# LuoweiZhou/VLP

Measured on NVIDIA H100. Metric: image_text_samples_per_sec, higher is better.
Workload: dtype bf16

## Files before the change

vlp_b200/csrc/common.cuh:

```cuda
#pragma once
#include <cuda.h>
#include <cuda_bf16.h>
#include <cuda_runtime.h>
#include <stdint.h>

#include "wgmma.cuh"

namespace vlpk {

__device__ __forceinline__ uint32_t smem_u32(const void* p) {
  return static_cast<uint32_t>(__cvta_generic_to_shared(p));
}

__device__ __forceinline__ uint32_t lane_id() { return threadIdx.x & 31u; }

__device__ __forceinline__ bool elect_one() {
  uint32_t pred = 0;
  asm volatile(
      "{\n\t"
      ".reg .pred P;\n\t"
      "elect.sync _|P, 0xffffffff;\n\t"
      "selp.u32 %0, 1, 0, P;\n\t"
      "}\n"
      : "=r"(pred));
  return pred != 0;
}

__device__ __forceinline__ void mbar_init(uint64_t* bar, uint32_t count) {
  asm volatile("mbarrier.init.shared::cta.b64 [%0], %1;" ::"r"(smem_u32(bar)), "r"(count) : "memory");
}
__device__ __forceinline__ void fence_mbar_init() {
  asm volatile("fence.mbarrier_init.release.cluster;" ::: "memory");
}
__device__ __forceinline__ void fence_proxy_async_smem() {
  asm volatile("fence.proxy.async.shared::cta;" ::: "memory");
}
__device__ __forceinline__ void mbar_arrive_expect_tx(uint64_t* bar, uint32_t bytes) {
  asm volatile("mbarrier.arrive.expect_tx.shared::cta.b64 _, [%0], %1;" ::"r"(smem_u32(bar)), "r"(bytes)
               : "memory");
}
__device__ __forceinline__ void mbar_arrive(uint64_t* bar) {
  asm volatile("mbarrier.arrive.shared::cta.b64 _, [%0];" ::"r"(smem_u32(bar)) : "memory");
}
__device__ __forceinline__ bool mbar_try_wait(uint64_t* bar, uint32_t parity) {
  uint32_t ok;
  asm volatile(
      "{\n\t"
      ".reg .pred P;\n\t"
      "mbarrier.try_wait.parity.shared::cta.b64 P, [%1], %2;\n\t"
      "selp.u32 %0, 1, 0, P;\n\t"
      "}\n"
      : "=r"(ok)
      : "r"(smem_u32(bar)), "r"(parity)
      : "memory");
  return ok != 0;
}
__device__ __forceinline__ void mbar_wait(uint64_t* bar, uint32_t parity) {
  uint32_t spins = 0;
  while (!mbar_try_wait(bar, parity)) {
    if (++spins > (1u << 28)) { __trap(); }
  }
}

__device__ __forceinline__ void pdl_launch_dependents() { asm volatile("griddepcontrol.launch_dependents;" ::: "memory"); }
__device__ __forceinline__ void pdl_wait() { asm volatile("griddepcontrol.wait;" ::: "memory"); }

__device__ __forceinline__ void tma_prefetch_desc(const CUtensorMap* m) {
  asm volatile("prefetch.tensormap [%0];" ::"l"(reinterpret_cast<uint64_t>(m)) : "memory");
}
__device__ __forceinline__ void tma_load_2d(void* dst, const CUtensorMap* m, uint64_t* bar, int c0, int c1) {
  asm volatile(
      "cp.async.bulk.tensor.2d.shared::cluster.global.tile.mbarrier::complete_tx::bytes [%0], [%1, {%3, %4}], [%2];"
      ::"r"(smem_u32(dst)), "l"(reinterpret_cast<uint64_t>(m)), "r"(smem_u32(bar)), "r"(c0), "r"(c1)
      : "memory");
}
__device__ __forceinline__ void tma_load_3d(void* dst, const CUtensorMap* m, uint64_t* bar, int c0, int c1,
                                            int c2) {
  asm volatile(
      "cp.async.bulk.tensor.3d.shared::cluster.global.tile.mbarrier::complete_tx::bytes [%0], [%1, {%3, %4, %5}], "
      "[%2];" ::"r"(smem_u32(dst)),
      "l"(reinterpret_cast<uint64_t>(m)), "r"(smem_u32(bar)), "r"(c0), "r"(c1), "r"(c2)
      : "memory");
}
__device__ __forceinline__ void tma_store_2d(const CUtensorMap* m, const void* src, int c0, int c1) {
  asm volatile("cp.async.bulk.tensor.2d.global.shared::cta.tile.bulk_group [%0, {%2, %3}], [%1];" ::"l"(
                   reinterpret_cast<uint64_t>(m)),
               "r"(smem_u32(src)), "r"(c0), "r"(c1)
               : "memory");
}
__device__ __forceinline__ void tma_store_3d(const CUtensorMap* m, const void* src, int c0, int c1, int c2) {
  asm volatile("cp.async.bulk.tensor.3d.global.shared::cta.tile.bulk_group [%0, {%2, %3, %4}], [%1];" ::"l"(
                   reinterpret_cast<uint64_t>(m)),
               "r"(smem_u32(src)), "r"(c0), "r"(c1), "r"(c2)
               : "memory");
}
__device__ __forceinline__ void tma_reduce_add_2d(const CUtensorMap* m, const void* src, int c0, int c1) {
  asm volatile("cp.reduce.async.bulk.tensor.2d.global.shared::cta.add.tile.bulk_group [%0, {%2, %3}], [%1];" ::"l"(
                   reinterpret_cast<uint64_t>(m)),
               "r"(smem_u32(src)), "r"(c0), "r"(c1)
               : "memory");
}
__device__ __forceinline__ void tma_reduce_add_3d(const CUtensorMap* m, const void* src, int c0, int c1, int c2) {
  asm volatile("cp.reduce.async.bulk.tensor.3d.global.shared::cta.add.tile.bulk_group [%0, {%2, %3, %4}], [%1];" ::"l"(
                   reinterpret_cast<uint64_t>(m)),
               "r"(smem_u32(src)), "r"(c0), "r"(c1), "r"(c2)
               : "memory");
}
__device__ __forceinline__ void tma_store_commit() { asm volatile("cp.async.bulk.commit_group;" ::: "memory"); }
template <int N>
__device__ __forceinline__ void tma_store_wait_read() {
  asm volatile("cp.async.bulk.wait_group.read %0;" ::"n"(N) : "memory");
}
template <int N>
__device__ __forceinline__ void tma_store_wait() {
  asm volatile("cp.async.bulk.wait_group %0;" ::"n"(N) : "memory");
}

__device__ __forceinline__ void wgmma_fence() { asm volatile("wgmma.fence.sync.aligned;" ::: "memory"); }
__device__ __forceinline__ void wgmma_commit() { asm volatile("wgmma.commit_group.sync.aligned;" ::: "memory"); }
template <int N>
__device__ __forceinline__ void wgmma_wait() {
  asm volatile("wgmma.wait_group.sync.aligned %0;" ::"n"(N) : "memory");
}
template <int N>
__device__ __forceinline__ void reg_fence(float (&d)[N]) {
#pragma unroll
  for (int i = 0; i < N; ++i) asm volatile("" : "+f"(d[i])::"memory");
}

__device__ __forceinline__ uint64_t wgmma_desc_sw128(uint32_t saddr, uint32_t lbo_bytes, uint32_t sbo_bytes) {
  uint64_t d = 0;
  d |= static_cast<uint64_t>((saddr & 0x3FFFFu) >> 4);
  d |= static_cast<uint64_t>((lbo_bytes >> 4) & 0x3FFFu) << 16;
  d |= static_cast<uint64_t>((sbo_bytes >> 4) & 0x3FFFu) << 32;
  d |= 1ull << 62;
  return d;
}

__device__ __forceinline__ uint32_t pack_bf16x2(float lo, float hi) {
  __nv_bfloat162 v = __floats2bfloat162_rn(lo, hi);
  return *reinterpret_cast<uint32_t*>(&v);
}
__device__ __forceinline__ float2 unpack_bf16x2(uint32_t u) {
  __nv_bfloat162 v = *reinterpret_cast<__nv_bfloat162*>(&u);
  return __bfloat1622float2(v);
}
__device__ __forceinline__ float bf16_round(float x) { return __bfloat162float(__float2bfloat16_rn(x)); }

__device__ __forceinline__ float fast_ex2(float x) {
  float y;
  asm("ex2.approx.ftz.f32 %0, %1;" : "=f"(y) : "f"(x));
  return y;
}
__device__ __forceinline__ float fast_rcp(float x) {
  float y;
  asm("rcp.approx.ftz.f32 %0, %1;" : "=f"(y) : "f"(x));
  return y;
}

__device__ __forceinline__ void gelu_and_grad(float x, float& g, float& d) {
  const float ax = fabsf(x);
  const float e = fast_ex2(-0.72134752044448170f * x * x);
  const float t = fast_rcp(fmaf(0.3275911f * 0.70710678118654752f, ax, 1.0f));
  float poly = fmaf(1.061405429f, t, -1.453152027f);
  poly = fmaf(poly, t, 1.421413741f);
  poly = fmaf(poly, t, -0.284496736f);
  poly = fmaf(poly, t, 0.254829592f);
  poly *= t;
  const float erf_abs = fmaf(-poly, e, 1.0f);
  const float cdf = 0.5f * (1.0f + copysignf(erf_abs, x));
  g = x * cdf;
  d = fmaf(x * 0.3989422804014327f, e, cdf);
}

struct Philox {
  __device__ __forceinline__ static uint4 gen(uint64_t seed, uint64_t ctr_hi, uint64_t ctr_lo) {
    uint32_t k0 = static_cast<uint32_t>(seed), k1 = static_cast<uint32_t>(seed >> 32);
    uint4 c = make_uint4(static_cast<uint32_t>(ctr_lo), static_cast<uint32_t>(ctr_lo >> 32),
                         static_cast<uint32_t>(ctr_hi), static_cast<uint32_t>(ctr_hi >> 32));
#pragma unroll
    for (int i = 0; i < 10; ++i) {
      const uint32_t hi0 = __umulhi(0xD2511F53u, c.x), lo0 = 0xD2511F53u * c.x;
      const uint32_t hi1 = __umulhi(0xCD9E8D57u, c.z), lo1 = 0xCD9E8D57u * c.z;
      c = make_uint4(hi1 ^ c.y ^ k0, lo1, hi0 ^ c.w ^ k1, lo0);
      k0 += 0x9E3779B9u;
      k1 += 0xBB67AE85u;
    }
    return c;
  }
};
__device__ __forceinline__ uint32_t dropout_keep8(uint64_t seed, uint64_t site, uint64_t idx8, uint32_t thresh16) {
  const uint4 r = Philox::gen(seed, site, idx8);
  uint32_t m = 0;
  m |= ((r.x & 0xFFFFu) >= thresh16) ? 1u : 0u;
  m |= ((r.x >> 16) >= thresh16) ? 2u : 0u;
  m |= ((r.y & 0xFFFFu) >= thresh16) ? 4u : 0u;
  m |= ((r.y >> 16) >= thresh16) ? 8u : 0u;
  m |= ((r.z & 0xFFFFu) >= thresh16) ? 16u : 0u;
  m |= ((r.z >> 16) >= thresh16) ? 32u : 0u;
  m |= ((r.w & 0xFFFFu) >= thresh16) ? 64u : 0u;
  m |= ((r.w >> 16) >= thresh16) ? 128u : 0u;
  return m;
}

struct DropoutCfg {
  float p;
  float scale;
  uint32_t thresh16;
  uint64_t seed;
  uint64_t site;
  const unsigned long long* seed_ptr;
  const unsigned char* bits;
};

__device__ __forceinline__ uint64_t drop_seed(const DropoutCfg& d) {
  return (d.p > 0.f && d.seed_ptr != nullptr) ? d.seed + *d.seed_ptr : d.seed;
}

__host__ inline DropoutCfg make_dropout(float p, uint64_t seed, uint64_t site,
                                        const unsigned long long* seed_ptr = nullptr) {
  DropoutCfg d;
  d.bits = nullptr;
  d.seed_ptr = seed_ptr;
  d.p = p;
  d.scale = p > 0.f ? 1.0f / (1.0f - p) : 1.0f;
  d.thresh16 = static_cast<uint32_t>(p * 65536.0f);
  d.seed = seed;
  d.site = site;
  return d;
}

}
```

vlp_b200/csrc/gemm.cu:

```cuda
#include "gemm.cuh"

#include <cstdlib>

#include "host.cuh"

namespace vlpk {

static constexpr int BM = 128;
static constexpr int BK = 64;
static constexpr int NUM_THREADS = 288;
static constexpr int STG_BYTES = 64 * 128;
static constexpr int SMEM_MAX = 232448;
static constexpr int BN = 128;

struct GemmTmaps {
  CUtensorMap a;
  CUtensorMap b[3];
  CUtensorMap d0;
  CUtensorMap d1;
};

struct GemmArgs {
  int M, N, K;
  int b_seg_rows;
  int splits;
  int split_slices;
  const __nv_bfloat16* bias[3];
  const __nv_bfloat16* aux;
  long long ld_aux;
  float relu_scale;
  DropoutCfg drop;
  float* colsum;
};

template <int STAGES>
struct SmemLayout {
  static constexpr int A_BYTES = BM * BK * 2;
  static constexpr int B_BYTES = BN * BK * 2;
  static constexpr int STAGE_BYTES = A_BYTES + B_BYTES;
  static constexpr int OFF_STG = STAGES * STAGE_BYTES;
  static constexpr int OFF_BAR = OFF_STG + 4 * STG_BYTES;
  static constexpr int NUM_BARS = 2 * STAGES;
  static constexpr int TOTAL = OFF_BAR + NUM_BARS * 8;
  static constexpr int DYN_BYTES = TOTAL + 1024;
  static_assert(DYN_BYTES <= SMEM_MAX, "shared memory budget exceeded");
};

struct StageCount {
  static constexpr int value = (SMEM_MAX - 1024 - 4 * STG_BYTES - 256) / (BM * BK * 2 + BN * BK * 2);
};

__device__ __forceinline__ void wg_bar_sync(int cw) {
  asm volatile("bar.sync %0, 128;" ::"r"(cw + 1) : "memory");
}

template <bool A_MN, bool B_MN, int EPI>
__global__ void __launch_bounds__(NUM_THREADS, 1)
gemm_kernel(const __grid_constant__ GemmTmaps tm, const GemmArgs args) {
  constexpr int STAGES = StageCount::value;
  using L = SmemLayout<STAGES>;
  extern __shared__ uint8_t smem_raw[];
  uint8_t* smem = reinterpret_cast<uint8_t*>((reinterpret_cast<uintptr_t>(smem_raw) + 1023) & ~uintptr_t(1023));

  uint64_t* bars = reinterpret_cast<uint64_t*>(smem + L::OFF_BAR);
  uint64_t* full_bar = bars;
  uint64_t* empty_bar = bars + STAGES;

  pdl_launch_dependents();
  const int wg = threadIdx.x >> 7;
  const int lane = threadIdx.x & 31;

  const int num_m = (args.M + BM - 1) / BM;
  const int num_n = (args.N + BN - 1) / BN;
  const int total_kb = (args.K + BK - 1) / BK;
  const int kb_per = (total_kb + args.splits - 1) / args.splits;
  const int num_work = num_m * num_n * args.splits;

  if (threadIdx.x == 0) {
    tma_prefetch_desc(&tm.a);
    tma_prefetch_desc(&tm.b[0]);
    tma_prefetch_desc(&tm.d0);
    for (int i = 0; i < STAGES; ++i) {
      mbar_init(&full_bar[i], 1);
      mbar_init(&empty_bar[i], 8);
    }
    fence_mbar_init();
  }
  __syncthreads();
  pdl_wait();

  if (wg == 2) {
    {
      int stage = 0;
      uint32_t phase = 0;
      for (int w = blockIdx.x; w < num_work; w += gridDim.x) {
        const int n_blk = w % num_n;
        const int m_blk = (w / num_n) % num_m;
        const int split = w / (num_n * num_m);
        const int kb0 = split * kb_per;
        const int kb1 = min(total_kb, kb0 + kb_per);
        const int m0 = m_blk * BM;
        for (int kb = kb0; kb < kb1; ++kb) {
          mbar_wait(&empty_bar[stage], phase ^ 1u);
          if (elect_one()) {
            uint8_t* sA = smem + stage * L::STAGE_BYTES;
            uint8_t* sB = sA + L::A_BYTES;
            mbar_arrive_expect_tx(&full_bar[stage], L::STAGE_BYTES);
            if (!A_MN) {
              tma_load_2d(sA, &tm.a, &full_bar[stage], kb * BK, m0);
            } else {
#pragma unroll
              for (int j = 0; j < BM / 64; ++j) tma_load_2d(sA + j * 8192, &tm.a, &full_bar[stage], m0 + j * 64, kb * BK);
            }
            if (!B_MN) {
              const int n0 = n_blk * BN;
              const int seg = n0 / args.b_seg_rows;
              tma_load_2d(sB, &tm.b[seg], &full_bar[stage], kb * BK, n0 - seg * args.b_seg_rows);
            } else {
              const int k0 = kb * BK;
              const int seg = k0 / args.b_seg_rows;
#pragma unroll
              for (int j = 0; j < BN / 64; ++j)
                tma_load_2d(sB + j * 8192, &tm.b[seg], &full_bar[stage], n_blk * BN + j * 64, k0 - seg * args.b_seg_rows);
            }
          }
          __syncwarp();
          if (++stage == STAGES) {
            stage = 0;
            phase ^= 1u;
          }
        }
      }
    }
  } else {
    const int cw = wg;
    const int t = threadIdx.x - 128 * wg;
    const int fr = (t >> 5) * 16 + (lane >> 2);
    const int fc = (lane & 3) * 2;
    const bool store_thread = (t == 0);
    const uint64_t dseed = drop_seed(args.drop);
    constexpr bool HAS_BIAS = !B_MN && (EPI == EPI_STORE || EPI == EPI_GELU || EPI == EPI_RELU);
    uint8_t* stg0 = smem + L::OFF_STG + cw * 2 * STG_BYTES;
    uint8_t* stg1 = stg0 + STG_BYTES;
    const uint32_t a_base = smem_u32(smem) + cw * 8192;
    const uint32_t b_base = smem_u32(smem) + L::A_BYTES;
    int stage = 0;
    uint32_t phase = 0;
    uint32_t box_seq = 0;
    float acc[BN / 2];
    for (int w = blockIdx.x; w < num_work; w += gridDim.x) {
      const int n_blk = w % num_n;
      const int m_blk = (w / num_n) % num_m;
      const int split = w / (num_n * num_m);
      const int kb0 = split * kb_per;
      const int kb1 = min(total_kb, kb0 + kb_per);
      const int n0 = n_blk * BN;
      const int m0 = m_blk * BM + cw * 64;

      for (int kb = kb0; kb < kb1; ++kb) {
        mbar_wait(&full_bar[stage], phase);
        const uint32_t sa = a_base + stage * L::STAGE_BYTES;
        const uint32_t sb = b_base + stage * L::STAGE_BYTES;
        reg_fence(acc);
        wgmma_fence();
#pragma unroll
        for (int k = 0; k < BK / 16; ++k) {
          const uint64_t adesc = A_MN ? wgmma_desc_sw128(sa + k * 2048, 8192, 1024) : wgmma_desc_sw128(sa + k * 32, 16, 1024);
          const uint64_t bdesc = B_MN ? wgmma_desc_sw128(sb + k * 2048, 8192, 1024) : wgmma_desc_sw128(sb + k * 32, 16, 1024);
          wgmma_m64n128k16_ss<A_MN ? 1 : 0, B_MN ? 1 : 0>(acc, adesc, bdesc, (kb > kb0 || k > 0) ? 1u : 0u);
        }
        wgmma_commit();
        wgmma_wait<0>();
        reg_fence(acc);
        if (lane == 0) mbar_arrive(&empty_bar[stage]);
        if (++stage == STAGES) {
          stage = 0;
          phase ^= 1u;
        }
      }

      if (EPI == EPI_REDUCE_F32) {
        constexpr int NBOX = BN / 32;
#pragma unroll
        for (int c = 0; c < NBOX; ++c) {
          uint8_t* stg = (box_seq & 1u) ? stg1 : stg0;
          if (store_thread) tma_store_wait_read<1>();
          wg_bar_sync(cw);
#pragma unroll
          for (int j = 0; j < 8; ++j) {
            const int i = c * 16 + 2 * j;
            const int r = fr + 8 * (j & 1), col = 8 * (j >> 1) + fc;
            *reinterpret_cast<float2*>(stg + r * 128 + (((col >> 2) ^ (r & 7)) << 4) + (col & 3) * 4) = make_float2(acc[i], acc[i + 1]);
          }
          fence_proxy_async_smem();
          wg_bar_sync(cw);
          if (store_thread) {
            tma_reduce_add_3d(&tm.d0, stg, n0 + c * 32, m0, args.split_slices ? split : 0);
            tma_store_commit();
          }
          ++box_seq;
        }
      } else {
        constexpr int NBOX = BN / 64;
        const __nv_bfloat16* bp = nullptr;
        int bias_off = 0;
        if (HAS_BIAS) {
          const int seg = n0 / args.b_seg_rows;
          bp = args.bias[seg];
          bias_off = seg * args.b_seg_rows;
        }
#pragma unroll
        for (int c = 0; c < NBOX; ++c) {
          uint8_t* stg = (EPI == EPI_GELU) ? stg0 : ((box_seq & 1u) ? stg1 : stg0);
          if (store_thread) {
            if (EPI == EPI_GELU) tma_store_wait_read<0>(); else tma_store_wait_read<1>();
          }
          wg_bar_sync(cw);
#pragma unroll
          for (int j = 0; j < 16; ++j) {
            const int i = c * 32 + 2 * j;
            const int r = fr + 8 * (j & 1), col = 8 * (j >> 1) + fc;
            const int n = n0 + c * 64 + col;
            const long long m = m0 + r;
            float v0 = acc[i], v1 = acc[i + 1];
            if (HAS_BIAS) {
              if (bp != nullptr && n < args.N) {
                const float2 bb = unpack_bf16x2(__ldg(reinterpret_cast<const unsigned int*>(bp + n - bias_off)));
                v0 += bb.x;
                v1 += bb.y;
              }
            }
            const int so = r * 128 + (((col >> 3) ^ (r & 7)) << 4) + (col & 7) * 2;
            if (EPI == EPI_GELU) {
              float g0, d0, g1, d1;
              gelu_and_grad(v0, g0, d0);
              gelu_and_grad(v1, g1, d1);
              *reinterpret_cast<uint32_t*>(stg0 + so) = pack_bf16x2(d0, d1);
              *reinterpret_cast<uint32_t*>(stg1 + so) = pack_bf16x2(g0, g1);
              continue;
            }
            if (EPI == EPI_RELU) {
              uint32_t keep = 0xFFu;
              if (args.drop.p > 0.f)
                keep = dropout_keep8(dseed, args.drop.site, (static_cast<uint64_t>(m) * args.N + (n - fc)) >> 3, args.drop.thresh16);
              v0 = fmaxf(v0, 0.f);
              v1 = fmaxf(v1, 0.f);
              v0 = ((keep >> fc) & 1u) ? v0 * args.drop.scale : 0.f;
              v1 = ((keep >> (fc + 1)) & 1u) ? v1 * args.drop.scale : 0.f;
            } else if (EPI == EPI_ADD || EPI == EPI_MUL || EPI == EPI_DRELU) {
              float2 x = make_float2(0.f, 0.f);
              if (m < args.M && n < args.N) x = unpack_bf16x2(__ldg(reinterpret_cast<const unsigned int*>(args.aux + m * args.ld_aux + n)));
              if (EPI == EPI_ADD) {
                v0 += x.x;
                v1 += x.y;
              } else if (EPI == EPI_MUL) {
                v0 *= x.x;
                v1 *= x.y;
              } else {
                v0 = x.x > 0.f ? v0 * args.relu_scale : 0.f;
                v1 = x.y > 0.f ? v1 * args.relu_scale : 0.f;
              }
            }
            *reinterpret_cast<uint32_t*>(stg + so) = pack_bf16x2(v0, v1);
          }
          fence_proxy_async_smem();
          wg_bar_sync(cw);
          if (store_thread) {
            tma_store_2d(&tm.d0, stg, n0 + c * 64, m0);
            if (EPI == EPI_GELU) tma_store_2d(&tm.d1, stg1, n0 + c * 64, m0);
            tma_store_commit();
          }
          if (EPI != EPI_GELU && args.colsum != nullptr) {
            const int col = t & 63, r0 = (t >> 6) * 32;
            float acc_c = 0.f;
#pragma unroll 8
            for (int rr = r0; rr < r0 + 32; ++rr) {
              const __nv_bfloat16 v = *reinterpret_cast<const __nv_bfloat16*>(stg + rr * 128 + (((col >> 3) ^ (rr & 7)) << 4) + (col & 7) * 2);
              acc_c += __bfloat162float(v);
            }
            if (n0 + c * 64 + col < args.N) atomicAdd(args.colsum + n0 + c * 64 + col, acc_c);
          }
          ++box_seq;
        }
      }
    }
    if (store_thread) tma_store_wait<0>();
  }
}

template <bool A_MN, bool B_MN, int EPI>
static int launch_inst(const GemmTmaps& tm, const GemmArgs& args, int num_work, cudaStream_t stream) {
  constexpr int STAGES = StageCount::value;
  using L = SmemLayout<STAGES>;
  auto kfn = gemm_kernel<A_MN, B_MN, EPI>;
  static bool attr_set = false;
  if (!attr_set) {
    VLPK_CUDA(cudaFuncSetAttribute(kfn, cudaFuncAttributeMaxDynamicSharedMemorySize, L::DYN_BYTES));
    attr_set = true;
  }
  const int max_ctas = gemm_sms();
  const int ctas = num_work < max_ctas ? num_work : max_ctas;
  LaunchScope scope(A_MN ? CAT_GEMM_WGRAD : (B_MN ? CAT_GEMM_DGRAD : CAT_GEMM_FWD), 2.0 * args.M * args.N * args.K, stream);
  VLPK_CUDA(launch_ex(kfn, dim3(ctas), dim3(NUM_THREADS), L::DYN_BYTES, stream, 1, tm, args));
  return 0;
}

static int dispatch(const GemmDesc& g, const GemmTmaps& tm, const GemmArgs& args, int num_work, cudaStream_t s) {
  if (!g.a_mn && !g.b_mn) {
    switch (g.epi) {
      case EPI_STORE: return launch_inst<false, false, EPI_STORE>(tm, args, num_work, s);
      case EPI_GELU: return launch_inst<false, false, EPI_GELU>(tm, args, num_work, s);
      case EPI_RELU: return launch_inst<false, false, EPI_RELU>(tm, args, num_work, s);
      default: break;
    }
  } else if (!g.a_mn && g.b_mn) {
    switch (g.epi) {
      case EPI_STORE: return launch_inst<false, true, EPI_STORE>(tm, args, num_work, s);
      case EPI_ADD: return launch_inst<false, true, EPI_ADD>(tm, args, num_work, s);
      case EPI_MUL: return launch_inst<false, true, EPI_MUL>(tm, args, num_work, s);
      case EPI_DRELU: return launch_inst<false, true, EPI_DRELU>(tm, args, num_work, s);
      case EPI_REDUCE_F32: return launch_inst<false, true, EPI_REDUCE_F32>(tm, args, num_work, s);
      default: break;
    }
  } else if (g.a_mn && g.b_mn) {
    if (g.epi == EPI_REDUCE_F32) return launch_inst<true, true, EPI_REDUCE_F32>(tm, args, num_work, s);
    if (g.epi == EPI_STORE) return launch_inst<true, true, EPI_STORE>(tm, args, num_work, s);
  }
  set_error("gemm: unsupported (a_mn=%d, b_mn=%d, epi=%d) combination", (int)g.a_mn, (int)g.b_mn, g.epi);
  return -1;
}

static double tile_cost(int M, int N, int total_kb, int splits, bool reduce) {
  const int num_m = (M + BM - 1) / BM;
  const int num_n = (N + BN - 1) / BN;
  const long long tiles = static_cast<long long>(num_m) * num_n * splits;
  const int slots = gemm_sms();
  const long long rounds = (tiles + slots - 1) / slots;
  const int kb_per = (total_kb + splits - 1) / splits;
  const double mainloop = kb_per * (128.0 + double(BN));
  const double epi = (reduce ? 3.0 : 1.5) * BN;
  return rounds * (mainloop + epi + 60.0);
}

int plan_gemm(const GemmDesc& g, int* bn_out, int* splits_out) {
  const int seg_rows = g.nseg > 1 ? g.b_seg_rows : (g.b_mn ? g.K : g.N);
  const int total_kb = (g.K + BK - 1) / BK;
  const bool reduce = (g.epi == EPI_REDUCE_F32);
  VLPK_CHECK_ARG(g.bn == 0 || g.bn == BN, "gemm: no valid tile configuration (bn=%d; tiles are %d wide)", g.bn, BN);
  VLPK_CHECK_ARG(g.nseg == 1 || seg_rows % (g.b_mn ? BK : BN) == 0, "gemm: segment rows %d not tile aligned", seg_rows);
  int splits = 1;
  if (reduce) {
    const int max_s = total_kb / 8 > 0 ? total_kb / 8 : 1;
    if (g.splits > 0) {
      splits = g.splits < max_s ? g.splits : max_s;
    } else {
      double best = 1e300;
      for (int s = 1; s <= max_s; ++s) {
        const double c = tile_cost(g.M, g.N, total_kb, s, reduce);
        if (c < best) {
          best = c;
          splits = s;
        }
      }
    }
  }
  if (splits > total_kb) splits = total_kb;
  {
    const int kb_per = (total_kb + splits - 1) / splits;
    splits = (total_kb + kb_per - 1) / kb_per;
  }
  *bn_out = BN;
  *splits_out = splits;
  return 0;
}

int launch_gemm(const GemmDesc& g, cudaStream_t stream) {
  VLPK_CHECK_ARG(g.M > 0 && g.N > 0 && g.K > 0, "gemm: empty problem M=%d N=%d K=%d", g.M, g.N, g.K);
  VLPK_CHECK_ARG(g.N % 8 == 0, "gemm: N=%d must be a multiple of 8", g.N);
  VLPK_CHECK_ARG(g.nseg >= 1 && g.nseg <= 3, "gemm: nseg=%d", g.nseg);
  const int seg_rows = g.nseg > 1 ? g.b_seg_rows : (g.b_mn ? g.K : g.N);
  const bool reduce = (g.epi == EPI_REDUCE_F32);
  VLPK_CHECK_ARG(g.splits <= 1 || reduce, "gemm: split-K needs EPI_REDUCE_F32");
  VLPK_CHECK_ARG(g.b_rows == 0 || (g.nseg == 1 && g.b_rows <= (g.b_mn ? g.K : g.N)), "gemm: b_rows=%d needs a single B segment", g.b_rows);

  int bn = BN, splits = 1;
  VLPK_TRY(plan_gemm(g, &bn, &splits));

  GemmTmaps tm;
  memset(&tm, 0, sizeof(tm));
  if (!g.a_mn) {
    VLPK_TRY(make_tmap_2d(&tm.a, TM_BF16, g.A, g.K, g.M, g.lda, BK, BM));
  } else {
    VLPK_TRY(make_tmap_2d(&tm.a, TM_BF16, g.A, g.M, g.K, g.lda, 64, BK));
  }
  for (int s = 0; s < g.nseg; ++s) {
    if (!g.b_mn) {
      const int rows = g.nseg > 1 ? seg_rows : (g.b_rows > 0 ? g.b_rows : g.N);
      VLPK_TRY(make_tmap_2d(&tm.b[s], TM_BF16, g.B[s], g.K, rows, g.ldb, BK, bn));
    } else {
      const int rows = g.nseg > 1 ? seg_rows : (g.b_rows > 0 ? g.b_rows : g.K);
      VLPK_TRY(make_tmap_2d(&tm.b[s], TM_BF16, g.B[s], g.N, rows, g.ldb, 64, BK));
    }
  }
  for (int s = g.nseg; s < 3; ++s) tm.b[s] = tm.b[0];
  if (reduce) {
    VLPK_CHECK_ARG(g.split_stride == 0 || (g.split_stride % 4 == 0 && g.split_stride >= static_cast<int64_t>(g.M) * g.ldd0),
                   "gemm: split_stride %lld must be a multiple of 4 and cover M x ldd0", (long long)g.split_stride);
    const uint64_t dims[3] = {static_cast<uint64_t>(g.N), static_cast<uint64_t>(g.M), static_cast<uint64_t>(g.split_stride ? splits : 1)};
    const uint64_t strides[2] = {static_cast<uint64_t>(g.ldd0) * 4,
                                 static_cast<uint64_t>(g.split_stride ? g.split_stride : static_cast<int64_t>(g.M) * g.ldd0) * 4};
    const uint32_t box[3] = {32, 64, 1};
    VLPK_TRY(make_tmap(&tm.d0, TM_F32, 3, g.D0, dims, strides, box));
    tm.d1 = tm.d0;
  } else {
    VLPK_TRY(make_tmap_2d(&tm.d0, TM_BF16, g.D0, g.N, g.M, g.ldd0, 64, 64));
    if (g.epi == EPI_GELU) {
      VLPK_CHECK_ARG(g.D1 != nullptr, "gemm: EPI_GELU needs D1");
      VLPK_TRY(make_tmap_2d(&tm.d1, TM_BF16, g.D1, g.N, g.M, g.ldd1, 64, 64));
    } else {
      tm.d1 = tm.d0;
    }
  }
  VLPK_CHECK_ARG(g.colsum == nullptr || (!reduce && g.epi != EPI_GELU), "gemm: colsum fusion is for single-output bf16 epilogues");
  if (g.epi == EPI_ADD || g.epi == EPI_MUL || g.epi == EPI_DRELU) {
    VLPK_CHECK_ARG(g.aux != nullptr && (g.ld_aux % 8) == 0 && (reinterpret_cast<uintptr_t>(g.aux) & 15u) == 0,
                   "gemm: aux must be 16-byte aligned with ld %% 8 == 0");
  }

  GemmArgs a;
  a.M = g.M;
  a.N = g.N;
  a.K = g.K;
  a.b_seg_rows = seg_rows;
  a.splits = splits;
  a.split_slices = (reduce && g.split_stride > 0) ? 1 : 0;
  for (int s = 0; s < 3; ++s) a.bias[s] = (s < g.nseg) ? g.bias[s] : nullptr;
  a.aux = g.aux;
  a.ld_aux = g.ld_aux;
  a.relu_scale = g.relu_scale;
  a.colsum = g.colsum;
  a.drop = g.drop;

  const int num_m = (g.M + BM - 1) / BM;
  const int num_n = (g.N + bn - 1) / bn;
  const int num_work = num_m * num_n * splits;
  return dispatch(g, tm, a, num_work, stream);
}

}
```

Measured before the change: 3810.

## Ping-pong two consumer warpgroups over whole tiles with register reallocation

```diff
diff --git a/vlp_b200/csrc/common.cuh b/vlp_b200/csrc/common.cuh
--- a/vlp_b200/csrc/common.cuh
+++ b/vlp_b200/csrc/common.cuh
@@ -121,6 +121,14 @@
 template <int N>
 __device__ __forceinline__ void wgmma_wait() {
   asm volatile("wgmma.wait_group.sync.aligned %0;" ::"n"(N) : "memory");
+}
+template <uint32_t N>
+__device__ __forceinline__ void setmaxnreg_inc() {
+  asm volatile("setmaxnreg.inc.sync.aligned.u32 %0;" ::"n"(N));
+}
+template <uint32_t N>
+__device__ __forceinline__ void setmaxnreg_dec() {
+  asm volatile("setmaxnreg.dec.sync.aligned.u32 %0;" ::"n"(N));
 }
 template <int N>
 __device__ __forceinline__ void reg_fence(float (&d)[N]) {
diff --git a/vlp_b200/csrc/gemm.cu b/vlp_b200/csrc/gemm.cu
--- a/vlp_b200/csrc/gemm.cu
+++ b/vlp_b200/csrc/gemm.cu
@@ -8,7 +8,10 @@
 
 static constexpr int BM = 128;
 static constexpr int BK = 64;
-static constexpr int NUM_THREADS = 288;
+static constexpr int NUM_THREADS = 384;
+static constexpr int PRODUCER_REGS = 40;
+static constexpr int MMA_REGS = 232;
+static_assert(128 * PRODUCER_REGS + 256 * MMA_REGS <= 65536, "register file of one SM exceeded");
 static constexpr int STG_BYTES = 64 * 128;
 static constexpr int SMEM_MAX = 232448;
 static constexpr int BN = 128;
@@ -50,8 +53,17 @@
   static constexpr int value = (SMEM_MAX - 1024 - 4 * STG_BYTES - 256) / (BM * BK * 2 + BN * BK * 2);
 };
 
+static constexpr int BAR_MAINLOOP = 3;
+static constexpr int BAR_EPILOGUE = 5;
+
 __device__ __forceinline__ void wg_bar_sync(int cw) {
   asm volatile("bar.sync %0, 128;" ::"r"(cw + 1) : "memory");
+}
+__device__ __forceinline__ void handoff_arrive(int bar) {
+  asm volatile("bar.arrive %0, 256;" ::"r"(bar) : "memory");
+}
+__device__ __forceinline__ void handoff_wait(int bar) {
+  asm volatile("bar.sync %0, 256;" ::"r"(bar) : "memory");
 }
 
 template <bool A_MN, bool B_MN, int EPI>
@@ -67,7 +79,7 @@
   uint64_t* empty_bar = bars + STAGES;
 
   pdl_launch_dependents();
-  const int wg = threadIdx.x >> 7;
+  const int wg = __shfl_sync(0xffffffffu, threadIdx.x >> 7, 0);
   const int lane = threadIdx.x & 31;
 
   const int num_m = (args.M + BM - 1) / BM;
@@ -82,7 +94,7 @@
     tma_prefetch_desc(&tm.d0);
     for (int i = 0; i < STAGES; ++i) {
       mbar_init(&full_bar[i], 1);
-      mbar_init(&empty_bar[i], 8);
+      mbar_init(&empty_bar[i], 4);
     }
     fence_mbar_init();
   }
@@ -90,6 +102,8 @@
   pdl_wait();
 
   if (wg == 2) {
+    setmaxnreg_dec<PRODUCER_REGS>();
+    if (threadIdx.x >= 256 + 32) return;
     {
       int stage = 0;
       uint32_t phase = 0;
@@ -133,6 +147,7 @@
       }
     }
   } else {
+    setmaxnreg_inc<MMA_REGS>();
     const int cw = wg;
     const int t = threadIdx.x - 128 * wg;
     const int fr = (t >> 5) * 16 + (lane >> 2);
@@ -142,147 +157,179 @@
     constexpr bool HAS_BIAS = !B_MN && (EPI == EPI_STORE || EPI == EPI_GELU || EPI == EPI_RELU);
     uint8_t* stg0 = smem + L::OFF_STG + cw * 2 * STG_BYTES;
     uint8_t* stg1 = stg0 + STG_BYTES;
-    const uint32_t a_base = smem_u32(smem) + cw * 8192;
+    const uint32_t a_base = smem_u32(smem);
     const uint32_t b_base = smem_u32(smem) + L::A_BYTES;
-    int stage = 0;
-    uint32_t phase = 0;
+    uint32_t ring_kb = 0;
     uint32_t box_seq = 0;
-    float acc[BN / 2];
-    for (int w = blockIdx.x; w < num_work; w += gridDim.x) {
+    float acc[2][BN / 2];
+    for (int i = 0, w = blockIdx.x; w < num_work; ++i, w += gridDim.x) {
       const int n_blk = w % num_n;
       const int m_blk = (w / num_n) % num_m;
       const int split = w / (num_n * num_m);
       const int kb0 = split * kb_per;
       const int kb1 = min(total_kb, kb0 + kb_per);
+      if ((i & 1) != cw) {
+        ring_kb += kb1 - kb0;
+        continue;
+      }
+      const bool has_prev = i > 0;
+      const bool has_next = w + gridDim.x < num_work;
       const int n0 = n_blk * BN;
-      const int m0 = m_blk * BM + cw * 64;
-
-      for (int kb = kb0; kb < kb1; ++kb) {
-        mbar_wait(&full_bar[stage], phase);
+
+      if (has_prev) handoff_wait(BAR_MAINLOOP + (cw ^ 1));
+      uint32_t prev_stage = 0;
+      for (int kb = kb0; kb < kb1; ++kb, ++ring_kb) {
+        const uint32_t stage = ring_kb % STAGES;
+        mbar_wait(&full_bar[stage], (ring_kb / STAGES) & 1u);
         const uint32_t sa = a_base + stage * L::STAGE_BYTES;
         const uint32_t sb = b_base + stage * L::STAGE_BYTES;
-        reg_fence(acc);
+        reg_fence(acc[0]);
+        reg_fence(acc[1]);
         wgmma_fence();
 #pragma unroll
         for (int k = 0; k < BK / 16; ++k) {
-          const uint64_t adesc = A_MN ? wgmma_desc_sw128(sa + k * 2048, 8192, 1024) : wgmma_desc_sw128(sa + k * 32, 16, 1024);
           const uint64_t bdesc = B_MN ? wgmma_desc_sw128(sb + k * 2048, 8192, 1024) : wgmma_desc_sw128(sb + k * 32, 16, 1024);
-          wgmma_m64n128k16_ss<A_MN ? 1 : 0, B_MN ? 1 : 0>(acc, adesc, bdesc, (kb > kb0 || k > 0) ? 1u : 0u);
+#pragma unroll
+          for (int h = 0; h < 2; ++h) {
+            const uint32_t sah = sa + h * 8192;
+            const uint64_t adesc = A_MN ? wgmma_desc_sw128(sah + k * 2048, 8192, 1024) : wgmma_desc_sw128(sah + k * 32, 16, 1024);
+            wgmma_m64n128k16_ss<A_MN ? 1 : 0, B_MN ? 1 : 0>(acc[h], adesc, bdesc, (kb > kb0 || k > 0) ? 1u : 0u);
+          }
         }
         wgmma_commit();
-        wgmma_wait<0>();
-        reg_fence(acc);
-        if (lane == 0) mbar_arrive(&empty_bar[stage]);
-        if (++stage == STAGES) {
-          stage = 0;
-          phase ^= 1u;
+        wgmma_wait<1>();
+        reg_fence(acc[0]);
+        reg_fence(acc[1]);
+        if (kb > kb0 && lane == 0) mbar_arrive(&empty_bar[prev_stage]);
+        prev_stage = stage;
+      }
+      if (has_next) handoff_arrive(BAR_MAINLOOP + cw);
+      wgmma_wait<0>();
+      reg_fence(acc[0]);
+      reg_fence(acc[1]);
+      if (lane == 0) mbar_arrive(&empty_bar[prev_stage]);
+
+      if (has_prev) handoff_wait(BAR_EPILOGUE + (cw ^ 1));
+      if (HAS_BIAS) {
+        const int seg = n0 / args.b_seg_rows;
+        const __nv_bfloat16* bp = seg == 0 ? args.bias[0] : (seg == 1 ? args.bias[1] : args.bias[2]);
+        if (bp != nullptr) {
+          bp -= seg * args.b_seg_rows;
+#pragma unroll
+          for (int j = 0; j < BN / 8; ++j) {
+            const int n = n0 + 8 * j + fc;
+            if (n < args.N) {
+              const float2 bb = unpack_bf16x2(__ldg(reinterpret_cast<const unsigned int*>(bp + n)));
+#pragma unroll
+              for (int h = 0; h < 2; ++h) {
+#pragma unroll
+                for (int q = 0; q < 2; ++q) {
+                  acc[h][4 * j + 2 * q] += bb.x;
+                  acc[h][4 * j + 2 * q + 1] += bb.y;
+                }
+              }
+            }
+          }
         }
       }
-
-      if (EPI == EPI_REDUCE_F32) {
-        constexpr int NBOX = BN / 32;
-#pragma unroll
-        for (int c = 0; c < NBOX; ++c) {
-          uint8_t* stg = (box_seq & 1u) ? stg1 : stg0;
-          if (store_thread) tma_store_wait_read<1>();
-          wg_bar_sync(cw);
-#pragma unroll
-          for (int j = 0; j < 8; ++j) {
-            const int i = c * 16 + 2 * j;
-            const int r = fr + 8 * (j & 1), col = 8 * (j >> 1) + fc;
-            *reinterpret_cast<float2*>(stg + r * 128 + (((col >> 2) ^ (r & 7)) << 4) + (col & 3) * 4) = make_float2(acc[i], acc[i + 1]);
-          }
-          fence_proxy_async_smem();
-          wg_bar_sync(cw);
-          if (store_thread) {
-            tma_reduce_add_3d(&tm.d0, stg, n0 + c * 32, m0, args.split_slices ? split : 0);
-            tma_store_commit();
-          }
-          ++box_seq;
+#pragma unroll 1
+      for (int h = 0; h < 2; ++h) {
+        const int m0 = m_blk * BM + h * 64;
+        float (&a)[BN / 2] = acc[0];
+        if (EPI == EPI_REDUCE_F32) {
+          constexpr int NBOX = BN / 32;
+#pragma unroll
+          for (int c = 0; c < NBOX; ++c) {
+            uint8_t* stg = (box_seq & 1u) ? stg1 : stg0;
+            if (store_thread) tma_store_wait_read<1>();
+            wg_bar_sync(cw);
+#pragma unroll
+            for (int j = 0; j < 8; ++j) {
+              const int i = c * 16 + 2 * j;
+              const int r = fr + 8 * (j & 1), col = 8 * (j >> 1) + fc;
+              *reinterpret_cast<float2*>(stg + r * 128 + (((col >> 2) ^ (r & 7)) << 4) + (col & 3) * 4) = make_float2(a[i], a[i + 1]);
+            }
+            fence_proxy_async_smem();
+            wg_bar_sync(cw);
+            if (store_thread) {
+              tma_reduce_add_3d(&tm.d0, stg, n0 + c * 32, m0, args.split_slices ? split : 0);
+              tma_store_commit();
+            }
+            ++box_seq;
+          }
+        } else {
+          constexpr int NBOX = BN / 64;
+#pragma unroll
+          for (int c = 0; c < NBOX; ++c) {
+            uint8_t* stg = (EPI == EPI_GELU) ? stg0 : ((box_seq & 1u) ? stg1 : stg0);
+            if (store_thread) {
+              if (EPI == EPI_GELU) tma_store_wait_read<0>(); else tma_store_wait_read<1>();
+            }
+            wg_bar_sync(cw);
+#pragma unroll
+            for (int j = 0; j < 16; ++j) {
+              const int i = c * 32 + 2 * j;
+              const int r = fr + 8 * (j & 1), col = 8 * (j >> 1) + fc;
+              const int n = n0 + c * 64 + col;
+              const long long m = m0 + r;
+              float v0 = a[i], v1 = a[i + 1];
+              const int so = r * 128 + (((col >> 3) ^ (r & 7)) << 4) + (col & 7) * 2;
+              if (EPI == EPI_GELU) {
+                float g0, d0, g1, d1;
+                gelu_and_grad(v0, g0, d0);
+                gelu_and_grad(v1, g1, d1);
+                *reinterpret_cast<uint32_t*>(stg0 + so) = pack_bf16x2(d0, d1);
+                *reinterpret_cast<uint32_t*>(stg1 + so) = pack_bf16x2(g0, g1);
+                continue;
+              }
+              if (EPI == EPI_RELU) {
+                uint32_t keep = 0xFFu;
+                if (args.drop.p > 0.f)
+                  keep = dropout_keep8(dseed, args.drop.site, (static_cast<uint64_t>(m) * args.N + (n - fc)) >> 3, args.drop.thresh16);
+                v0 = fmaxf(v0, 0.f);
+                v1 = fmaxf(v1, 0.f);
+                v0 = ((keep >> fc) & 1u) ? v0 * args.drop.scale : 0.f;
+                v1 = ((keep >> (fc + 1)) & 1u) ? v1 * args.drop.scale : 0.f;
+              } else if (EPI == EPI_ADD || EPI == EPI_MUL || EPI == EPI_DRELU) {
+                float2 x = make_float2(0.f, 0.f);
+                if (m < args.M && n < args.N) x = unpack_bf16x2(__ldg(reinterpret_cast<const unsigned int*>(args.aux + m * args.ld_aux + n)));
+                if (EPI == EPI_ADD) {
+                  v0 += x.x;
+                  v1 += x.y;
+                } else if (EPI == EPI_MUL) {
+                  v0 *= x.x;
+                  v1 *= x.y;
+                } else {
+                  v0 = x.x > 0.f ? v0 * args.relu_scale : 0.f;
+                  v1 = x.y > 0.f ? v1 * args.relu_scale : 0.f;
+                }
+              }
+              *reinterpret_cast<uint32_t*>(stg + so) = pack_bf16x2(v0, v1);
+            }
+            fence_proxy_async_smem();
+            wg_bar_sync(cw);
+            if (store_thread) {
+              tma_store_2d(&tm.d0, stg, n0 + c * 64, m0);
+              if (EPI == EPI_GELU) tma_store_2d(&tm.d1, stg1, n0 + c * 64, m0);
+              tma_store_commit();
+            }
+            if (EPI != EPI_GELU && args.colsum != nullptr) {
+              const int col = t & 63, r0 = (t >> 6) * 32;
+              float acc_c = 0.f;
+#pragma unroll 8
+              for (int rr = r0; rr < r0 + 32; ++rr) {
+                const __nv_bfloat16 v = *reinterpret_cast<const __nv_bfloat16*>(stg + rr * 128 + (((col >> 3) ^ (rr & 7)) << 4) + (col & 7) * 2);
+                acc_c += __bfloat162float(v);
+              }
+              if (n0 + c * 64 + col < args.N) atomicAdd(args.colsum + n0 + c * 64 + col, acc_c);
+            }
+            ++box_seq;
+          }
         }
-      } else {
-        constexpr int NBOX = BN / 64;
-        const __nv_bfloat16* bp = nullptr;
-        int bias_off = 0;
-        if (HAS_BIAS) {
-          const int seg = n0 / args.b_seg_rows;
-          bp = args.bias[seg];
-          bias_off = seg * args.b_seg_rows;
-        }
-#pragma unroll
-        for (int c = 0; c < NBOX; ++c) {
-          uint8_t* stg = (EPI == EPI_GELU) ? stg0 : ((box_seq & 1u) ? stg1 : stg0);
-          if (store_thread) {
-            if (EPI == EPI_GELU) tma_store_wait_read<0>(); else tma_store_wait_read<1>();
-          }
-          wg_bar_sync(cw);
-#pragma unroll
-          for (int j = 0; j < 16; ++j) {
-            const int i = c * 32 + 2 * j;
-            const int r = fr + 8 * (j & 1), col = 8 * (j >> 1) + fc;
-            const int n = n0 + c * 64 + col;
-            const long long m = m0 + r;
-            float v0 = acc[i], v1 = acc[i + 1];
-            if (HAS_BIAS) {
-              if (bp != nullptr && n < args.N) {
-                const float2 bb = unpack_bf16x2(__ldg(reinterpret_cast<const unsigned int*>(bp + n - bias_off)));
-                v0 += bb.x;
-                v1 += bb.y;
-              }
-            }
-            const int so = r * 128 + (((col >> 3) ^ (r & 7)) << 4) + (col & 7) * 2;
-            if (EPI == EPI_GELU) {
-              float g0, d0, g1, d1;
-              gelu_and_grad(v0, g0, d0);
-              gelu_and_grad(v1, g1, d1);
-              *reinterpret_cast<uint32_t*>(stg0 + so) = pack_bf16x2(d0, d1);
-              *reinterpret_cast<uint32_t*>(stg1 + so) = pack_bf16x2(g0, g1);
-              continue;
-            }
-            if (EPI == EPI_RELU) {
-              uint32_t keep = 0xFFu;
-              if (args.drop.p > 0.f)
-                keep = dropout_keep8(dseed, args.drop.site, (static_cast<uint64_t>(m) * args.N + (n - fc)) >> 3, args.drop.thresh16);
-              v0 = fmaxf(v0, 0.f);
-              v1 = fmaxf(v1, 0.f);
-              v0 = ((keep >> fc) & 1u) ? v0 * args.drop.scale : 0.f;
-              v1 = ((keep >> (fc + 1)) & 1u) ? v1 * args.drop.scale : 0.f;
-            } else if (EPI == EPI_ADD || EPI == EPI_MUL || EPI == EPI_DRELU) {
-              float2 x = make_float2(0.f, 0.f);
-              if (m < args.M && n < args.N) x = unpack_bf16x2(__ldg(reinterpret_cast<const unsigned int*>(args.aux + m * args.ld_aux + n)));
-              if (EPI == EPI_ADD) {
-                v0 += x.x;
-                v1 += x.y;
-              } else if (EPI == EPI_MUL) {
-                v0 *= x.x;
-                v1 *= x.y;
-              } else {
-                v0 = x.x > 0.f ? v0 * args.relu_scale : 0.f;
-                v1 = x.y > 0.f ? v1 * args.relu_scale : 0.f;
-              }
-            }
-            *reinterpret_cast<uint32_t*>(stg + so) = pack_bf16x2(v0, v1);
-          }
-          fence_proxy_async_smem();
-          wg_bar_sync(cw);
-          if (store_thread) {
-            tma_store_2d(&tm.d0, stg, n0 + c * 64, m0);
-            if (EPI == EPI_GELU) tma_store_2d(&tm.d1, stg1, n0 + c * 64, m0);
-            tma_store_commit();
-          }
-          if (EPI != EPI_GELU && args.colsum != nullptr) {
-            const int col = t & 63, r0 = (t >> 6) * 32;
-            float acc_c = 0.f;
-#pragma unroll 8
-            for (int rr = r0; rr < r0 + 32; ++rr) {
-              const __nv_bfloat16 v = *reinterpret_cast<const __nv_bfloat16*>(stg + rr * 128 + (((col >> 3) ^ (rr & 7)) << 4) + (col & 7) * 2);
-              acc_c += __bfloat162float(v);
-            }
-            if (n0 + c * 64 + col < args.N) atomicAdd(args.colsum + n0 + c * 64 + col, acc_c);
-          }
-          ++box_seq;
-        }
-      }
+#pragma unroll
+        for (int i = 0; i < BN / 2; ++i) acc[0][i] = acc[1][i];
+      }
+      if (has_next) handoff_arrive(BAR_EPILOGUE + cw);
     }
     if (store_thread) tma_store_wait<0>();
   }
```

New measurement: 3862, median of 6. 1.01x the previous value.
